# Lounes78/matcha-tts

Hardware: AMD Instinct MI355X
Metric: mel-frames/sec + RTF, text->wav @10 ODE steps, LJSpeech model, 1/2/4/8 GPU (higher is better)
Workload: dtype bf16

## Files before the change

include/matcha_hip.h:

```cpp
#ifndef MATCHA_HIP_H
#define MATCHA_HIP_H

#include <stddef.h>
#include <stdint.h>

#ifdef __cplusplus
extern "C" {
#endif

#define MT_DTYPE_F32 0
#define MT_DTYPE_BF16 1
#define MT_SOLVER_EULER 0
#define MT_SOLVER_MIDPOINT 1

const char* mt_last_error(void);
int mt_abi_version(void);
int mt_build_experiments(void);
int mt_sched_count(void);
int mt_sched_get(int i, int* rec, int* wait, int* wait_first, int cap);

typedef struct mt_encoder mt_encoder;
int mt_encoder_create(int n_vocab, int n_channels, int filter_channels, int n_heads, int n_layers, int kernel_size,
                      int n_spks, int spk_emb_dim, int dp_filter_channels, int dp_kernel_size, int prenet, int dtype,
                      mt_encoder** out);
// ... 132 lines not shown
int mtt_softmax_bwd(const float* p, const float* dp, const float* kmask, const float* qmask, int BH, int H, int Tq,
                    int Tk, float scale, float* ds, void* stream);
int mtt_rope(float* x, int B, int T, int H, int dh, int d, const float* theta, int inverse, void* stream);
int mtt_embed_fwd(const int64_t* ids, size_t ntok, const float* table, int C, float scale, float* out, void* stream);
int mtt_embed_bwd(const int64_t* ids, size_t ntok, const float* dout, int V, int C, float scale, float* dtable,
                  void* stream);
int mtt_adam(float* p, const float* g, float* m, float* v, size_t n, const float* gscale, float lr, float beta1,
             float beta2, float eps, int step, void* stream);
int mtt_clip_factor(const float* sumsq, float max_norm, float inv_world, float* out, float* norm_out, void* stream);
int mtt_unscale(float* g, size_t n, float inv_scale, float* found, float* scratch, void* stream);

size_t mt_op_conv1d_workspace_bytes(int dtype, int cin, int cout, int k, int stride, int transposed);
int mt_op_conv1d(int dtype, const void* x, int B, int Tin, int cin, const float* W, const float* bias,
                 int cout, int k, int stride, int pad, int dil, int transposed, float slope, void* y,
                 int Tout, void* ws, size_t ws_bytes, void* stream);
int mt_op_conv1d_tile(int variant, int dtype, const void* x, int B, int Tin, int cin, const float* W,
                      const float* bias, int cout, int k, int stride, int pad, int dil, int transposed,
                      float slope, void* y, int Tout, void* ws, size_t ws_bytes, void* stream);
size_t mt_op_vconv_workspace_bytes(int cin, int cout, int k);
int mt_op_vconv(const void* x, int B, int L, int cin, const float* W, const float* bias, int cout, int k, int dil,
                int ef, const void* resid, void* y, void* y2, float slope, float div, const int32_t* lens, int pack,
                void* ws, size_t ws_bytes, void* stream);
int mt_vconv_set_rbconv(int enable);
int mt_vconv_set_ct(int enable);
int mt_vpair_set_kernels(int mask);
int mt_vocoder_set_post_fold(int enable);
int mt_vconv_set_actin(int enable);
int mt_ffn_set(int enable);
int mt_ffn_set_min_frames(int frames);
int mt_decoder_set_kernels(int mask);
int mt_op_attention(int dtype, const void* qkv, const float* mask, void* out, int B, int T, int heads,
                    void* stream);

#define MT_PROBE_RBFUSE_C64 1
#define MT_PROBE_RBFUSE_C32 2
#define MT_PROBE_VCONV 3
#define MT_PROBE_VCONV_DEC 4
int mt_probe_start(int site, int max_launches);
int mt_probe_pause(int paused);
int mt_probe_detail(int cap, double* ms, double* flops, double* bytes, int* tags);
int mt_probe_stop(int* launches, double* total_ms, double* flops, double* bytes, double peak_flops, double peak_bw,
                  double* roof_ms);

#define MT_VCONV_LOG_FIELDS 11
int mt_vconv_log_start(int capacity);
int mt_vconv_log_stop(int32_t* records, int capacity);
// ... 7 lines not shown
```

matcha-tts_amd/csrc/mt_capi.hip:

```cpp
#include <string.h>

#include <new>

#include "../../include/matcha_hip.h"
#include "mt_ffn.h"
#include "mt_model.h"
#include "mt_vconv.h"
#include "mt_vpair.h"
#include "mt_probe.h"
#include "mt_train.h"

namespace mt {
const char* last_error();
int denoise(const float* audio, int B, int L, const float* bias_spec, float strength, float* out, void* ws,
            size_t ws_bytes, hipStream_t st, const int* lens = nullptr, int lmul = 1);
size_t denoise_workspace_bytes(int B, int L);
int vconv_exp_flags();
int rbconv_exp_flags();
int ffn_exp_flags();
int vpair_exp_flags();
int stft_magnitude(const float* audio, int B, int L, float* mag, hipStream_t st);
int log_mel(const float* audio, int B, int L, const float* basis, float mean, float stdv, float* mel, hipStream_t st);
}

// ... 351 lines not shown
  mt::ConvArgs a = mt::gemm_args(g, (const char*)ws, B, Tin);
  MT_REQUIRE(a.Tout == Tout, "op_conv1d: Tout %d != expected %d", Tout, a.Tout);
  a.x0 = x;
  a.y = y;
  a.slope = slope;
  return mt::launch_conv_op(dtype, slope >= 0.f ? mt::PF_LRELU : 0, a, st, variant);
}
int mt_op_conv1d(int dtype, const void* x, int B, int Tin, int cin, const float* W, const float* bias,
                 int cout, int k, int stride, int pad, int dil, int transposed, float slope, void* y, int Tout,
                 void* ws, size_t ws_bytes, void* stream) {
  return mt_op_conv1d_tile(-1, dtype, x, B, Tin, cin, W, bias, cout, k, stride, pad, dil, transposed, slope, y,
                           Tout, ws, ws_bytes, stream);
}
size_t mt_op_vconv_workspace_bytes(int cin, int cout, int k) {
  mt::Packer pk;
  mt::GemmW g = mt::make_conv(cout, cin, k, 1, 0, 1, {0}, 1, 2, pk);
  pk.take(mt::vconv_packed_bytes(cin, cout, k));
  pk.take(256);
  pk.take(4096);
  (void)g;
  return pk.off;
}
int mt_vconv_set_rbconv(int enable) { return mt::rbconv_set(enable); }
int mt_vconv_set_ct(int enable) { return mt::vconv_set_ct(enable); }
int mt_ffn_set(int enable) { return mt::ffn_set(enable); }
int mt_vconv_set_actin(int enable) { return mt::rbconv_actin_set(enable); }
int mt_ffn_set_min_frames(int frames) { return mt::ffn_set_min_frames(frames); }
int mt_decoder_set_kernels(int mask) { return mt::dec_set_kernels(mask); }
int mt_op_vconv(const void* x, int B, int L, int cin, const float* W, const float* bias, int cout, int k, int dil,
                int ef, const void* resid, void* y, void* y2, float slope, float div, const int32_t* lens, int pack,
                void* ws, size_t ws_bytes, void* stream) {
  MT_REQUIRE(x && W && bias && y && ws, "op_vconv: null argument");
  MT_REQUIRE(mt::vconv_supported(cin, cout, k, dil, 1), "op_vconv: unsupported conv %dx%d k%d d%d", cin, cout, k, dil);
  hipStream_t st = (hipStream_t)stream;
  mt::Packer pk;
  mt::GemmW g = mt::make_conv(cout, cin, k, 1, dil * (k - 1) / 2, dil, {0}, 1, 2, pk);
  const size_t v_off = pk.take(mt::vconv_packed_bytes(cin, cout, k));
  const size_t z_off = pk.take(256);
  const size_t t_off = pk.take(4096);
  MT_REQUIRE(ws_bytes >= pk.off, "op_vconv: workspace %zu < %zu", ws_bytes, pk.off);
  const float* params[2] = {W, bias};
  char* P = (char*)ws;
  int rc;
  if (pack) {
    if ((rc = mt::pack_gemm(g, MT_DTYPE_BF16, params, P, st))) return rc;
    if ((rc = mt::vconv_repack(P + g.w_off, g.Mpad, g.taps, g.cin_pad, cin, cout, P + v_off, st))) return rc;
// ... 155 lines not shown
```

matcha-tts_amd/csrc/mt_ragged.h:

```cpp
#pragma once
#include "mt_common.h"

namespace mt {

constexpr int RAG_MAXB = 512;
constexpr int RAG_LDS = 2 * RAG_MAXB * 4;

__device__ __forceinline__ void rag_build(int* tc, int* lv, const int* lens, int lmul, int Lpad, int extra, int cap,
                                          int B, int BN, int tid) {
  if (tid >= 64) return;
  const int per = (B + 63) >> 6, b0 = tid * per;
  int s = 0;
  for (int i = 0; i < per; ++i) {
    const int b = b0 + i;
    if (b < B) {
      const int L = min(max(lens[b] * lmul, 0), Lpad);
      const int nc = min(max(L + extra, 0), cap);
      s += (nc + BN - 1) / BN;
    }
  }
  int x = s;
#pragma unroll
  for (int o = 1; o < 64; o <<= 1) {
    const int v = __shfl_up(x, o, 64);
    if (tid >= o) x += v;
  }
  int run = x - s;
  for (int i = 0; i < per; ++i) {
    const int b = b0 + i;
    if (b < B) {
      const int L = min(max(lens[b] * lmul, 0), Lpad);
      const int nc = min(max(L + extra, 0), cap);
      run += (nc + BN - 1) / BN;
      tc[b] = run;
      lv[b] = L;
    }
  }
}

__device__ __forceinline__ int rag_find(const int* tc, int B, int r) {
  int lo = 0, hi = B - 1;
  while (lo < hi) {
    const int mid = (lo + hi) >> 1;
    if (tc[mid] > r) hi = mid;
    else lo = mid + 1;
  }
  return lo;
}

__device__ __forceinline__ int rag_first(const int* tc, int b) { return b > 0 ? tc[b - 1] : 0; }

struct RagTile {
  int b, n0, lv;
};
struct RagWalk {
// ... 13 lines not shown
```

matcha-tts_amd/csrc/mt_rbconv.hip:

```cpp
#include <algorithm>
#include <cstdlib>
#include <type_traits>

#include "mt_probe.h"
#include "mt_ragged.h"
#include "mt_ts.h"
#include "mt_vconv.h"

#ifndef RB_ACTIN_NV
#define RB_ACTIN_NV 0
#endif

#ifndef RB_RAGWALK
#define RB_RAGWALK 1
#endif

#ifndef RB_EPI_AT
#define RB_EPI_AT 2
#endif

#ifndef RB_DMA_AT
#define RB_DMA_AT 1
#endif

#ifndef RB_BUF
#define RB_BUF 7
#endif

#ifndef RB_LMAX
#define RB_LMAX 1
#endif

#ifndef RB_EXP
#define RB_EXP 0
#endif

namespace mt {

namespace {
constexpr int RBM = 128, RBN = 256, RNT = 512;
constexpr int RWSLOT = RBM * 128;
constexpr int RNW = 4;
constexpr int RXROWS = RBN + 64;
constexpr int RXBUF = RXROWS * 128;
constexpr int RX_OFF = RNW * RWSLOT;
constexpr int RBIAS_OFF = RX_OFF + 2 * RXBUF;
constexpr int RRAG_OFF = RBIAS_OFF + 256 * 4;
constexpr int RLDS = RRAG_OFF + RAG_LDS;
static_assert(RLDS <= 160 * 1024, "LDS budget");
constexpr int RFN = 4, RWNC = 64;

template <int LW>
struct RbStage {
// ... 136 lines not shown
      for (int i = 0; i < XPW; ++i) {
        if (i * TX / XPW != part) continue;
        const int j = wave + LW * i;
        buf_lds16(xr, (unsigned)(xlane + (f0 + 8 * j) * C * 2), 0u, dst + j * 1024);
      }
    } else {
#pragma unroll
      for (int i = 0; i < XPW; ++i) {
        if (i * TX / XPW != part) continue;
        const int j = wave + LW * i;
        const int r = 8 * j + lrow;
        const int q = lp ^ (r & 6);
        const int f = f0 + r;
        const bool ok = r < R && f >= 0 && f < Lx;
        const char* src = ok ? xb + (size_t)f * C * 2 + q * 16 : reinterpret_cast<const char*>(a.zero) + q * 16;
        rb_glds16(src, dst + j * 1024);
      }
    }
  };

  f32x4 acc[4][RFN];

  const int g4 = lane >> 4, l16 = lane & 15;
  auto swap16 = [](uint32_t& x, uint32_t& y) {
    const auto r = __builtin_amdgcn_permlane16_swap(x, y, false, false);
    x = r[0];
    y = r[1];
  };
  const int ch16 = wm * 64 + (g4 & 1) * 16 + (g4 >> 1) * 8;
  u32x4 rv[2][RFN], yv[2][RFN];
  auto epi_loads = [&](const Tile& tl) __attribute__((always_inline)) {
    const size_t rowbase = (size_t)tl.b * L;
#pragma unroll
    for (int fp = 0; fp < 2; ++fp)
#pragma unroll
      for (int fn = 0; fn < RFN; ++fn) {
        const int n = min(tl.n0 + wn * RWNC + fn * 16 + l16, L - 1);
        const size_t o = (rowbase + n) * C + tl.m0 + ch16 + fp * 32;
        if constexpr ((RB_EXP & 1) != 0) {
          rv[fp][fn] = yv[fp][fn] = u32x4{(uint32_t)o, 0u, 0u, 0u};
          continue;
        }
        if constexpr ((EF & VE_RESID) != 0) rv[fp][fn] = *reinterpret_cast<const u32x4*>(a.resid + o);
        if constexpr ((EF & VE_ACCUM) != 0) yv[fp][fn] = *reinterpret_cast<const u32x4*>(a.y + o);
      }
  };
  auto epilogue = [&](const Tile& tl, bool real) __attribute__((always_inline)) {
    const unsigned ylim = (unsigned)L * (unsigned)(C * 2) - (unsigned)(tl.m0 * 2);
    const auto yr = buf_rsrc(a.y + (size_t)tl.b * L * C + tl.m0, ylim);
    const auto y2r = buf_rsrc(((EF & VE_DUAL) ? a.y2 : a.y) + (size_t)tl.b * L * C + tl.m0, ylim);
#pragma unroll
    for (int fp = 0; fp < 2; ++fp)
#pragma unroll
      for (int fn = 0; fn < RFN; ++fn) {
        uint32_t rx0 = 0, rx1 = 0, ry0 = 0, ry1 = 0, yx0 = 0, yx1 = 0, yy0 = 0, yy1 = 0;
        if constexpr ((EF & VE_RESID) != 0) {
          rx0 = rv[fp][fn][0], rx1 = rv[fp][fn][1], ry0 = rv[fp][fn][2], ry1 = rv[fp][fn][3];
          swap16(rx0, ry0);
          swap16(rx1, ry1);
        }
        if constexpr ((EF & VE_ACCUM) != 0) {
          yx0 = yv[fp][fn][0], yx1 = yv[fp][fn][1], yy0 = yv[fp][fn][2], yy1 = yv[fp][fn][3];
          swap16(yx0, yy0);
          swap16(yx1, yy1);
        }
        uint32_t o1[2][2], o2[2][2];
#pragma unroll
        for (int h = 0; h < 2; ++h) {
          const int fm = 2 * fp + h;
          const int m = tl.m0 + wm * 64 + fm * 16 + 4 * g4;
          const f32x4 bias4 = *reinterpret_cast<const f32x4*>(smem + RBIAS_OFF + 4 * m);
          const uint32_t rr[2] = {h ? ry0 : rx0, h ? ry1 : rx1};
          const uint32_t yy[2] = {h ? yy0 : yx0, h ? yy1 : yx1};
#pragma unroll
          for (int u = 0; u < 2; ++u) {
            f32x2 v = f32x2{acc[fm][fn][2 * u], acc[fm][fn][2 * u + 1]} + f32x2{bias4[2 * u], bias4[2 * u + 1]};
            if constexpr ((EF & VE_RESID) != 0) v = v + unpk_bf16(rr[u]);
            if constexpr ((EF & VE_ACCUM) != 0) v = unpk_bf16(yy[u]) + v;
            if constexpr ((EF & VE_DIV) != 0) v = f32x2{div_rn(v.x, a.div, 1.f / a.div), div_rn(v.y, a.div, 1.f / a.div)};
            const uint32_t rb = pk_bf16(v);
            uint32_t av = 0u;
            if constexpr (RB_LMAX) av = (EF & VE_ACT) ? lrelu_pk_f(v, a.slope) : (EF & VE_DUAL) ? lrelu_pk(rb, a.slope) : 0u;
            else av = (EF & VE_ACT) ? lrelu_pk_f_sel(v, a.slope) : (EF & VE_DUAL) ? lrelu_pk_sel(rb, a.slope) : 0u;
            o1[h][u] = (EF & VE_ACT) ? av : rb;
            o2[h][u] = av;
          }
        }
        swap16(o1[0][0], o1[1][0]);
        swap16(o1[0][1], o1[1][1]);
        const int n = tl.n0 + wn * RWNC + fn * 16 + l16;
        if constexpr ((RB_BUF & 4) != 0) {
          const unsigned vo = (unsigned)((n * C + ch16 + fp * 32) * 2);
          if constexpr ((EF & VE_Y2ONLY) == 0)
            __builtin_amdgcn_raw_buffer_store_b128(u32x4{o1[0][0], o1[0][1], o1[1][0], o1[1][1]}, yr, vo, 0, 0);
          if constexpr ((EF & VE_DUAL) != 0 && (RB_EXP & 2) == 0) {
            swap16(o2[0][0], o2[1][0]);
            swap16(o2[0][1], o2[1][1]);
            __builtin_amdgcn_raw_buffer_store_b128(u32x4{o2[0][0], o2[0][1], o2[1][0], o2[1][1]}, y2r, vo, 0, 0);
          }
          continue;
        }
        const bool ok = real && n < L;
        const size_t o = ((size_t)tl.b * L + n) * C + tl.m0 + ch16 + fp * 32;
        if constexpr ((EF & VE_Y2ONLY) == 0)
          *reinterpret_cast<u32x4*>(ok ? a.y + o : a.trash + 8 * lane) = u32x4{o1[0][0], o1[0][1], o1[1][0], o1[1][1]};
        if constexpr ((EF & VE_DUAL) != 0 && (RB_EXP & 2) == 0) {
          swap16(o2[0][0], o2[1][0]);
          swap16(o2[0][1], o2[1][1]);
          *reinterpret_cast<u32x4*>(ok ? a.y2 + o : a.trash + 8 * lane) = u32x4{o2[0][0], o2[0][1], o2[1][0], o2[1][1]};
        }
      }
  };

  struct Frag {
    bf16x8 A[4], B[RFN];
  };
  const int ha = l16 & 6;
  const char* pa0 = smem + (wm * 64 + l16) * 128;
  const int rbl = wn * RWNC + l16;
  auto read_frag = [&](Frag& F, int ks, int slot, int xbuf, int tap) __attribute__((always_inline)) {
    int lb = rbl, la = 0;
    asm volatile("" : "+v"(lb), "+v"(la));
    const char* pa = pa0 + la + slot * RWSLOT;
    const int rb0 = lb + tap * dil;
    const int hb = rb0 & 6;
    const char* pb = smem + RX_OFF + xbuf * RXBUF + rb0 * 128;
    const int oa = ((ks * 4 + g4) ^ ha) * 16, ob = ((ks * 4 + g4) ^ hb) * 16;
#pragma unroll
    for (int f = 0; f < 4; ++f) F.A[f] = *reinterpret_cast<const bf16x8*>(pa + f * 2048 + oa);
#pragma unroll
    for (int f = 0; f < RFN; ++f) F.B[f] = *reinterpret_cast<const bf16x8*>(pb + f * 2048 + ob);
  };
  auto act_pass = [&](int buf) __attribute__((always_inline)) {
// ... 223 lines not shown
```

matcha-tts_amd/csrc/mt_vconv.h:

```cpp
#pragma once
#include <type_traits>

#include "mt_common.h"

namespace mt {

enum : int {
  VE_RESID = 1,
  VE_ACCUM = 2,
  VE_DIV = 4,
  VE_ACT = 8,
  VE_DUAL = 16,
  VE_LN = 32,
  VE_SNAKE = 64,
  VE_MASK = 128,
  VE_GNSTATS = 256,
  VE_ROWSTATS = 512,
  VE_LNP = 1024,
  VE_RELU = 2048,
  VE_PMASK = 4096,
  VE_ACTIN = 16384,
  VE_Y2ONLY = 32768,
  VE_POST = 131072,
  VE_SPLIT6 = 65536,
// ... 128 lines not shown
  int xcd_tiles;
};

__device__ __forceinline__ float2 ln_merge4(f32x4 p01, f32x4 p23, float eps) {
#pragma clang fp contract(off)
  const float mean = 0.25f * ((p01[0] + p01[2]) + (p23[0] + p23[2]));
  const float d0 = p01[0] - mean, d1 = p01[2] - mean, d2 = p23[0] - mean, d3 = p23[2] - mean;
  const float m2 = (p01[1] + p01[3]) + (p23[1] + p23[3]) + 64.f * ((d0 * d0 + d1 * d1) + (d2 * d2 + d3 * d3));
  return float2{mean, rsqrtf(m2 * (1.f / 256.f) + eps)};
}

int vconv_gn_parts(int B, int L, int M);
int vconv_gn_parts_max(int L);
int vconv_gnres_min_frames();

bool vconv_supported(int cin, int cout, int k, int dil, int stride);
size_t vconv_packed_bytes(int cin, int cout, int k);
int vconv_repack(const void* src, int Mpad0, int taps, int cin_pad, int cin, int cout, void* dst, hipStream_t st,
                 int cin_src = -1);
int launch_vconv(int ef, const VConvArgs& a, hipStream_t st);
bool rbconv_handles(int ef, const VConvArgs& a);
int launch_rbconv(int ef, const VConvArgs& a, int G, hipStream_t st);
int rbconv_set(int enable);
int rbconv_actin_set(int enable);
int rbconv_actin_on();
int vconv_set_ct(int enable);
int vconv_path_id();
bool vconv_supported_f32(int cin, int cout, int k, int stride);
size_t vconv_packed_bytes_f32(int cin, int cout, int k);
int vconv_repack_f32(const void* src, int Mpad0, int taps, int cin_pad, int cin, int cout, void* dst, hipStream_t st);
size_t vconv_packed_bytes_split6(int cin, int cout, int k);
int vconv_repack_split6(const void* src, int Mpad0, int taps, int cin_pad, int cin, int cout, void* dst, hipStream_t st);
__device__ __forceinline__ void split3_bf16(float v, bf16& h1, bf16& h2, bf16& h3) {
  h1 = (bf16)v;
  const float r1 = v - (float)h1;
  h2 = (bf16)r1;
  h3 = (bf16)(r1 - (float)h2);
}
int vconv_repack_s2(const void* src, int cin_pad, int C, int cout, void* dst, hipStream_t st);
int vconv_wsum(const void* img, int cin, int taps, int cout, float* wsum, hipStream_t st);

}
```

matcha-tts_amd/csrc/mt_vconv.hip:

```cpp
#include <algorithm>
#include <climits>
#include <cstdlib>
#include <type_traits>

#include "mt_misc.h"
#include "mt_probe.h"
#include "mt_ragged.h"
#include "mt_vconv.h"

namespace mt {

namespace {
constexpr int BN = 256, NT = 512;
constexpr int MMAX = 1024;
constexpr int BMP = 64;
template <int BM_, bool K1_, int NPAR_, int BN_ = BN>
struct VT {
  static constexpr int BM = BM_, TBN = BN_;
  static constexpr int WAVES_M = BM / 64, WAVES_N = 8 / WAVES_M;
  static constexpr int WNC = TBN / WAVES_N;
  static constexpr int FN = WNC / 16;
  static_assert(WNC % 16 == 0, "a wave covers whole 16-frame fragments");
  static constexpr int WSLOT = BM * 128;
  static constexpr int NWW = BM / 64;
// ... 1250 lines not shown
  if (tf != BN) ntiles = (long)a.B * ((a.L + tf - 1) / tf) * (a.Mpad / BM);
  const int G = (int)std::min<long>(ntiles, cu_count());
  a.xcd_tiles = a.xcd_tiles && ntiles <= 3L * G;
  MT_REQUIRE(!(ef & VE_GNSTATS) || a0.gn_parts == 0 || a0.gn_parts == ((a.L + tf - 1) / tf) * (8 / (BM / 64)),
             "vconv: caller expects %d GroupNorm partial slots, the launch writes a different count", a0.gn_parts);
  {
    const int bn = k1 ? tf1 : (BM == 64 ? (bm64_128 ? 128 : 384) : tf);
    const int rec[VCLOG_FIELDS] = {ef, BM, bn, (int)k1, (int)ntiles, G, a.taps, a.M, a.cin, a.B, a.L};
    vclog_record(rec);
#if defined(VCONV_TS)
    ts_assign(a, rec);
#endif
  }
  const double flops = 2.0 * a.M * a.cin * a.taps * (double)a.B * a.Lout;
  const double bytes = 2.0 * a.B * ((double)a.L * a.cin + (double)a.Lout * a.M) + 2.0 * a.M * a.cin * a.taps;
  const int site = a.probe ? a.probe : PROBE_VCONV;
  const bool probed = !k1 && site > 0;
  if ((ef & VE_Y2ONLY) && !(!k1 && !placed && BM == 128 && rbconv_handles(ef, a))) ef &= ~VE_Y2ONLY;
  MT_REQUIRE(!(ef & VE_ACTIN) || (!k1 && !placed && BM == 128 && rbconv_handles(ef, a)),
             "vconv: VE_ACTIN launch not taken by mt_rbconv (cin %d M %d k %d d %d B %d): stage_actin and the launch "
             "arguments disagree", a.cin, a.M, a.taps, a.dil, a.B);
  if (!k1 && !placed && BM == 128 && rbconv_handles(ef, a)) {
    if (probed) probe_begin(site, st);
    const int rc = launch_rbconv(ef, a, G, st);
    if (rc) return rc;
    if (probed) probe_end(site, st, flops, bytes, PROBE_TAG_RBCONV);
    return 0;
  }
  if (probed) probe_begin(site, st);
#define MT_VCASE(E)                                                                                \
  case E:                                                                                          \
    if (BM == 128) hipLaunchKernelGGL((vconv_kernel<E, 128, false>), dim3(G), dim3(NT), 0, st, a); \
    else hipLaunchKernelGGL((vconv_kernel<E, 64, false, BN64>), dim3(G), dim3(NT), 0, st, a);     \
    break;
#define MT_VCASE_H(E)                                                                                  \
  case E:                                                                                              \
    if (tf == 128) hipLaunchKernelGGL((vconv_kernel<E, 128, false, 128>), dim3(G), dim3(NT), 0, st, a); \
    else if (tf == 192) hipLaunchKernelGGL((vconv_kernel<E, 128, false, 192>), dim3(G), dim3(NT), 0, st, a); \
    else if (BM == 128) hipLaunchKernelGGL((vconv_kernel<E, 128, false>), dim3(G), dim3(NT), 0, st, a); \
    else hipLaunchKernelGGL((vconv_kernel<E, 64, false, BN64>), dim3(G), dim3(NT), 0, st, a);          \
    break;
#define MT_VCASE1(E)                                                                                    \
  case E:                                                                                               \
    if (tf1 == 128) {                                                                                   \
      if (BM == 128) hipLaunchKernelGGL((vconv_kernel<E, 128, true, 128>), dim3(G), dim3(NT), 0, st, a); \
      else hipLaunchKernelGGL((vconv_kernel<E, 64, true, 128>), dim3(G), dim3(NT), 0, st, a);           \
    } else if (tf1 == 192) {                \
// ... 101 lines not shown
```

matcha-tts_amd/matcha_hip/_lib.py:

```python
from __future__ import annotations

import ctypes
import os
from ctypes import POINTER, c_char_p, c_double, c_float, c_int, c_int64, c_size_t, c_uint, c_void_p

PKG_DIR = os.path.dirname(os.path.dirname(os.path.abspath(__file__)))
LIB_PATH = os.path.join(PKG_DIR, "libmatcha_hip.so")

DTYPE_F32 = 0
DTYPE_BF16 = 1
SOLVER_EULER = 0
SOLVER_MIDPOINT = 1

P = c_void_p

SIGNATURES = {
    "mt_last_error": (c_char_p, []),
    "mt_abi_version": (c_int, []),
    "mt_build_experiments": (c_int, []),
    "mt_sched_count": (c_int, []),
    "mt_sched_get": (c_int, [c_int, P, P, P, c_int]),
    "mt_encoder_create": (c_int, [c_int, c_int, c_int, c_int, c_int, c_int, c_int, c_int, c_int, c_int, c_int, c_int,
                                  POINTER(c_void_p)]),
    "mt_encoder_destroy": (None, [P]),
# ... 43 lines not shown
    "mt_vocoder_ragged_supported": (c_int, [P]),
    "mt_durations": (c_int, [P, P, c_float, c_int, c_int, P, P, P, P]),
    "mt_durations_scaled": (c_int, [P, P, P, c_int, c_int, P, P, P, P]),
    "mt_alignment": (c_int, [P, P, c_int, c_int, c_int, P, c_int, P, P, P, P]),
    "mt_denorm_crop": (c_int, [P, P, P, c_int, c_int, c_int, c_int, P, P]),
    "mt_denoise_workspace_bytes": (c_size_t, [c_int, c_int]),
    "mt_denoise": (c_int, [P, c_int, c_int, P, c_float, P, P, c_size_t, P]),
    "mt_denoise_ragged": (c_int, [P, c_int, c_int, P, c_int, P, c_float, P, P, c_size_t, P]),
    "mt_maximum_path_workspace_bytes": (c_size_t, [c_int, c_int, c_int]),
    "mt_decoder_step_times_workspace_bytes": (c_size_t, [P, c_int, c_int]),
    "mt_decoder_step_times": (c_int, [P, P, P, P, P, P, P, c_int, c_int, P, P, c_size_t, P]),
    "mt_maximum_path": (c_int, [P, P, P, c_int, c_int, c_int, P, P, c_size_t, P]),
    "mt_stft_magnitude": (c_int, [P, c_int, c_int, P, P]),
    "mt_log_mel": (c_int, [P, c_int, c_int, P, c_float, c_float, P, P]),
    "mt_op_conv1d_workspace_bytes": (c_size_t, [c_int, c_int, c_int, c_int, c_int, c_int]),
    "mt_op_conv1d": (c_int, [c_int, P, c_int, c_int, c_int, P, P, c_int, c_int, c_int, c_int, c_int,
                             c_int, c_float, P, c_int, P, c_size_t, P]),
    "mt_op_conv1d_tile": (c_int, [c_int, c_int, P, c_int, c_int, c_int, P, P, c_int, c_int, c_int, c_int, c_int,
                                  c_int, c_float, P, c_int, P, c_size_t, P]),
    "mt_op_vconv_workspace_bytes": (c_size_t, [c_int, c_int, c_int]),
    "mt_op_vconv": (c_int, [P, c_int, c_int, c_int, P, P, c_int, c_int, c_int, c_int, P, P, P, c_float, c_float,
                            P, c_int, P, c_size_t, P]),
    "mt_vconv_set_rbconv": (c_int, [c_int]),
    "mt_vconv_set_ct": (c_int, [c_int]),
    "mt_vpair_set_kernels": (c_int, [c_int]),
    "mt_vocoder_set_post_fold": (c_int, [c_int]),
    "mt_ffn_set": (c_int, [c_int]),
    "mt_vconv_set_actin": (c_int, [c_int]),
    "mt_ffn_set_min_frames": (c_int, [c_int]),
    "mt_decoder_set_kernels": (c_int, [c_int]),
    "mt_op_attention": (c_int, [c_int, P, P, P, c_int, c_int, c_int, P]),
    "mt_probe_start": (c_int, [c_int, c_int]),
    "mt_probe_pause": (c_int, [c_int]),
    "mt_probe_detail": (c_int, [c_int, P, P, P, P]),
    "mt_probe_stop": (c_int, [P, P, P, P, c_double, c_double, P]),
    "mtt_gemm": (c_int, [c_int, c_int, c_int, c_int, c_int, c_float, P, c_int, c_int64, P, c_int, c_int64, c_float,
                         P, c_int, c_int64, c_int, P, P, P, c_size_t, P]),
    "mtt_gemm_ex": (c_int, [c_int, c_int, c_int, c_int, c_int, c_int, c_float, P, c_int, c_int64, P, c_int, c_int64,
                            c_float, P, c_int, c_int64, c_int, P, P, P, c_size_t, P]),
    "mtt_gemm_workspace_bytes": (c_size_t, [c_int, c_int, c_int, c_int]),
    "mtt_im2col": (c_int, [P, P, c_int, c_int, c_int, c_int, c_int, c_int, c_int, c_int, P, P]),
    "mtt_col2im": (c_int, [P, P, c_int, c_int, c_int, c_int, c_int, c_int, c_int, c_int, P, c_int, P]),
    "mtt_ew": (c_int, [c_int, c_size_t, P, P, P, P, c_float, c_float, c_size_t, c_size_t, c_size_t, c_size_t,
                       c_size_t, c_size_t, c_int, P]),
    "mtt_copy_cols": (c_int, [P, c_int, c_int, P, c_int, c_int, c_int, c_int, c_int, P]),
    "mtt_seq_mask": (c_int, [P, c_int, c_int, P, P]),
# ... 75 lines not shown
```

matcha-tts_amd/matcha_hip/runtime.py:

```python
from __future__ import annotations

import math
import numbers
import time
from ctypes import byref, c_char_p, c_int, c_int64, c_void_p, create_string_buffer
from typing import Dict, List, Optional, Tuple

import torch

from ._lib import (DTYPE_BF16, DTYPE_F32, SOLVER_EULER, SOLVER_MIDPOINT, HipPathError, check, lib,
                   ptr, stream_handle)

_DTYPES = {"fp32": DTYPE_F32, "float32": DTYPE_F32, "f32": DTYPE_F32,
           "bf16": DTYPE_BF16, "bfloat16": DTYPE_BF16,
           "fp32x3": DTYPE_F32}


def dtype_code(precision: str) -> int:
    try:
        return _DTYPES[precision]
    except KeyError:
        raise ValueError(f"precision must be one of {sorted(set(_DTYPES))}, got {precision!r}")


# ... 594 lines not shown
    return int(lib().mt_vocoder_set_post_fold(int(bool(enable))))


def set_ffn(mode) -> int:
    return int(lib().mt_ffn_set(int(mode)))


def set_ffn_min_frames(frames: int) -> int:
    return int(lib().mt_ffn_set_min_frames(int(frames)))


def set_decoder_kernels(mask: int) -> int:
    return int(lib().mt_decoder_set_kernels(int(mask)))


def set_rbconv_actin(enable: bool) -> bool:
    return bool(lib().mt_vconv_set_actin(int(bool(enable))))


def set_rbconv(enable: bool) -> bool:
    return bool(lib().mt_vconv_set_rbconv(int(bool(enable))))


def op_attention(qkv: torch.Tensor, mask: torch.Tensor, heads: int, precision="fp32") -> torch.Tensor:
    require_gpu(qkv, mask, what="op_attention")
    dt = dtype_code(precision)
    et = torch.bfloat16 if dt == DTYPE_BF16 else torch.float32
    qkv = qkv.to(et).contiguous()
    B, T, _ = qkv.shape
    out = torch.empty((B, T, heads * 64), dtype=et, device=qkv.device)
    mask = f32c(mask.reshape(B, T))
    check(lib().mt_op_attention(dt, ptr(qkv), ptr(mask), ptr(out), B, T, heads, stream_handle(qkv.device)),
          "op_attention")
    return out


PROBE_RBFUSE_C64, PROBE_RBFUSE_C32, PROBE_VCONV, PROBE_VCONV_DEC = 1, 2, 3, 4


def probe_start(site: int, max_launches: int) -> None:
    check(lib().mt_probe_start(int(site), int(max_launches)), "probe_start")


def probe_pause(paused: bool) -> None:
    check(lib().mt_probe_pause(int(bool(paused))), "probe_pause")

# ... 2 lines not shown


def probe_detail(cap: int = 4096) -> List[Dict[str, float]]:
    from ctypes import c_double
    ms, fl, by, tg = (c_double * cap)(), (c_double * cap)(), (c_double * cap)(), (c_int * cap)()
    n = lib().mt_probe_detail(int(cap), ms, fl, by, tg)
    if n < 0:
        check(n, "probe_detail")
    return [{"ms": ms[i], "flops": fl[i], "bytes": by[i], "kind": PROBE_TAGS[tg[i]]} for i in range(n)]


def probe_stop(peak_flops: float = 2.5e15, peak_bw: float = 8.0e12) -> Dict[str, float]:
    from ctypes import c_double
    n, ms, fl, by, roof = c_int(0), c_double(0), c_double(0), c_double(0), c_double(0)
    check(lib().mt_probe_stop(byref(n), byref(ms), byref(fl), byref(by), float(peak_flops), float(peak_bw),
                              byref(roof)), "probe_stop")
    return {"launches": n.value, "ms": ms.value, "flops": fl.value, "bytes": by.value, "roof_ms": roof.value}


VCONV_LOG_FIELDS = ("ef", "bm", "bn", "k1", "ntiles", "grid", "taps", "M", "cin", "B", "L")
PROJ_LOG = 0x20000
UNI_LOG_PART, UNI_LOG_VEC, UNI_LOG_APPLY = 0x40000, 0x80000, 0xC0000
FFN_LOG = 0x400000
LOG_CONV, LOG_AUX = 1, 2


def vconv_log_select(families: int) -> int:
    return int(lib().mt_vconv_log_select(int(families)))


def vconv_log_start(capacity: int = 65536) -> None:
    check(lib().mt_vconv_log_start(int(capacity)), "vconv_log_start")


def vconv_log_stop(capacity: int = 65536) -> List[Dict[str, int]]:
    buf = (c_int * (capacity * len(VCONV_LOG_FIELDS)))()
    n = lib().mt_vconv_log_stop(buf, int(capacity))
    k = len(VCONV_LOG_FIELDS)
    return [dict(zip(VCONV_LOG_FIELDS, buf[i * k:(i + 1) * k])) for i in range(n)]
```

Before: 815,700.

## Add weight-stationary persistent conv kernel for 128-channel vocoder resblock convs

Adds a new persistent HIP kernel that keeps the full 128x128xK conv weights in registers across tiles and loops over ragged time tiles per CU. It double-buffers input rows in LDS and overlaps the next tile's load with the current compute. By default it is used for k=7 resblock convs with residual, accumulate or dual epilogues. The epilogue is factored into a shared header, and ragged tile counts gain an optional rounding. This is meant to remove repeated weight loads and per-tile launch overhead, at the cost of high register pressure and one block per CU.

Result: no change. 818,300 (median of 6 runs) (+0.3%).

```diff
diff --git a/include/matcha_hip.h b/include/matcha_hip.h
--- a/include/matcha_hip.h
+++ b/include/matcha_hip.h
@@ -178,6 +178,7 @@
                 int ef, const void* resid, void* y, void* y2, float slope, float div, const int32_t* lens, int pack,
                 void* ws, size_t ws_bytes, void* stream);
 int mt_vconv_set_rbconv(int enable);
+int mt_vconv_set_wsconv(int mode);
 int mt_vconv_set_ct(int enable);
 int mt_vpair_set_kernels(int mask);
 int mt_vocoder_set_post_fold(int enable);
diff --git a/matcha-tts_amd/csrc/mt_capi.hip b/matcha-tts_amd/csrc/mt_capi.hip
--- a/matcha-tts_amd/csrc/mt_capi.hip
+++ b/matcha-tts_amd/csrc/mt_capi.hip
@@ -397,6 +397,7 @@
   return pk.off;
 }
 int mt_vconv_set_rbconv(int enable) { return mt::rbconv_set(enable); }
+int mt_vconv_set_wsconv(int mode) { return mt::wsconv_set(mode); }
 int mt_vconv_set_ct(int enable) { return mt::vconv_set_ct(enable); }
 int mt_ffn_set(int enable) { return mt::ffn_set(enable); }
 int mt_vconv_set_actin(int enable) { return mt::rbconv_actin_set(enable); }
diff --git a/matcha-tts_amd/csrc/mt_ragged.h b/matcha-tts_amd/csrc/mt_ragged.h
--- a/matcha-tts_amd/csrc/mt_ragged.h
+++ b/matcha-tts_amd/csrc/mt_ragged.h
@@ -7,7 +7,7 @@
 constexpr int RAG_LDS = 2 * RAG_MAXB * 4;
 
 __device__ __forceinline__ void rag_build(int* tc, int* lv, const int* lens, int lmul, int Lpad, int extra, int cap,
-                                          int B, int BN, int tid) {
+                                          int B, int BN, int tid, int round = 1) {
   if (tid >= 64) return;
   const int per = (B + 63) >> 6, b0 = tid * per;
   int s = 0;
@@ -15,7 +15,7 @@
     const int b = b0 + i;
     if (b < B) {
       const int L = min(max(lens[b] * lmul, 0), Lpad);
-      const int nc = min(max(L + extra, 0), cap);
+      const int nc = min((max(L + extra, 0) + round - 1) / round * round, cap);
       s += (nc + BN - 1) / BN;
     }
   }
@@ -30,7 +30,7 @@
     const int b = b0 + i;
     if (b < B) {
       const int L = min(max(lens[b] * lmul, 0), Lpad);
-      const int nc = min(max(L + extra, 0), cap);
+      const int nc = min((max(L + extra, 0) + round - 1) / round * round, cap);
       run += (nc + BN - 1) / BN;
       tc[b] = run;
       lv[b] = L;
diff --git a/matcha-tts_amd/csrc/mt_rbconv.hip b/matcha-tts_amd/csrc/mt_rbconv.hip
--- a/matcha-tts_amd/csrc/mt_rbconv.hip
+++ b/matcha-tts_amd/csrc/mt_rbconv.hip
@@ -4,6 +4,7 @@
 
 #include "mt_probe.h"
 #include "mt_ragged.h"
+#include "mt_rbepi.h"
 #include "mt_ts.h"
 #include "mt_vconv.h"
 
@@ -25,10 +26,6 @@
 
 #ifndef RB_BUF
 #define RB_BUF 7
-#endif
-
-#ifndef RB_LMAX
-#define RB_LMAX 1
 #endif
 
 #ifndef RB_EXP
@@ -211,11 +208,6 @@
   f32x4 acc[4][RFN];
 
   const int g4 = lane >> 4, l16 = lane & 15;
-  auto swap16 = [](uint32_t& x, uint32_t& y) {
-    const auto r = __builtin_amdgcn_permlane16_swap(x, y, false, false);
-    x = r[0];
-    y = r[1];
-  };
   const int ch16 = wm * 64 + (g4 & 1) * 16 + (g4 >> 1) * 8;
   u32x4 rv[2][RFN], yv[2][RFN];
   auto epi_loads = [&](const Tile& tl) __attribute__((always_inline)) {
@@ -242,62 +234,24 @@
     for (int fp = 0; fp < 2; ++fp)
 #pragma unroll
       for (int fn = 0; fn < RFN; ++fn) {
-        uint32_t rx0 = 0, rx1 = 0, ry0 = 0, ry1 = 0, yx0 = 0, yx1 = 0, yy0 = 0, yy1 = 0;
-        if constexpr ((EF & VE_RESID) != 0) {
-          rx0 = rv[fp][fn][0], rx1 = rv[fp][fn][1], ry0 = rv[fp][fn][2], ry1 = rv[fp][fn][3];
-          swap16(rx0, ry0);
-          swap16(rx1, ry1);
-        }
-        if constexpr ((EF & VE_ACCUM) != 0) {
-          yx0 = yv[fp][fn][0], yx1 = yv[fp][fn][1], yy0 = yv[fp][fn][2], yy1 = yv[fp][fn][3];
-          swap16(yx0, yy0);
-          swap16(yx1, yy1);
-        }
-        uint32_t o1[2][2], o2[2][2];
-#pragma unroll
-        for (int h = 0; h < 2; ++h) {
-          const int fm = 2 * fp + h;
-          const int m = tl.m0 + wm * 64 + fm * 16 + 4 * g4;
-          const f32x4 bias4 = *reinterpret_cast<const f32x4*>(smem + RBIAS_OFF + 4 * m);
-          const uint32_t rr[2] = {h ? ry0 : rx0, h ? ry1 : rx1};
-          const uint32_t yy[2] = {h ? yy0 : yx0, h ? yy1 : yx1};
-#pragma unroll
-          for (int u = 0; u < 2; ++u) {
-            f32x2 v = f32x2{acc[fm][fn][2 * u], acc[fm][fn][2 * u + 1]} + f32x2{bias4[2 * u], bias4[2 * u + 1]};
-            if constexpr ((EF & VE_RESID) != 0) v = v + unpk_bf16(rr[u]);
-            if constexpr ((EF & VE_ACCUM) != 0) v = unpk_bf16(yy[u]) + v;
-            if constexpr ((EF & VE_DIV) != 0) v = f32x2{div_rn(v.x, a.div, 1.f / a.div), div_rn(v.y, a.div, 1.f / a.div)};
-            const uint32_t rb = pk_bf16(v);
-            uint32_t av = 0u;
-            if constexpr (RB_LMAX) av = (EF & VE_ACT) ? lrelu_pk_f(v, a.slope) : (EF & VE_DUAL) ? lrelu_pk(rb, a.slope) : 0u;
-            else av = (EF & VE_ACT) ? lrelu_pk_f_sel(v, a.slope) : (EF & VE_DUAL) ? lrelu_pk_sel(rb, a.slope) : 0u;
-            o1[h][u] = (EF & VE_ACT) ? av : rb;
-            o2[h][u] = av;
-          }
-        }
-        swap16(o1[0][0], o1[1][0]);
-        swap16(o1[0][1], o1[1][1]);
+        u32x4 out1, out2;
+        rb_epi_pair<EF>(a, acc[2 * fp][fn], acc[2 * fp + 1][fn], rv[fp][fn], yv[fp][fn],
+                        smem + RBIAS_OFF + 4 * (tl.m0 + wm * 64 + fp * 32 + 4 * g4), out1, out2);
         const int n = tl.n0 + wn * RWNC + fn * 16 + l16;
         if constexpr ((RB_BUF & 4) != 0) {
           const unsigned vo = (unsigned)((n * C + ch16 + fp * 32) * 2);
           if constexpr ((EF & VE_Y2ONLY) == 0)
-            __builtin_amdgcn_raw_buffer_store_b128(u32x4{o1[0][0], o1[0][1], o1[1][0], o1[1][1]}, yr, vo, 0, 0);
-          if constexpr ((EF & VE_DUAL) != 0 && (RB_EXP & 2) == 0) {
-            swap16(o2[0][0], o2[1][0]);
-            swap16(o2[0][1], o2[1][1]);
-            __builtin_amdgcn_raw_buffer_store_b128(u32x4{o2[0][0], o2[0][1], o2[1][0], o2[1][1]}, y2r, vo, 0, 0);
-          }
+            __builtin_amdgcn_raw_buffer_store_b128(out1, yr, vo, 0, 0);
+          if constexpr ((EF & VE_DUAL) != 0 && (RB_EXP & 2) == 0)
+            __builtin_amdgcn_raw_buffer_store_b128(out2, y2r, vo, 0, 0);
           continue;
         }
         const bool ok = real && n < L;
         const size_t o = ((size_t)tl.b * L + n) * C + tl.m0 + ch16 + fp * 32;
         if constexpr ((EF & VE_Y2ONLY) == 0)
-          *reinterpret_cast<u32x4*>(ok ? a.y + o : a.trash + 8 * lane) = u32x4{o1[0][0], o1[0][1], o1[1][0], o1[1][1]};
-        if constexpr ((EF & VE_DUAL) != 0 && (RB_EXP & 2) == 0) {
-          swap16(o2[0][0], o2[1][0]);
-          swap16(o2[0][1], o2[1][1]);
-          *reinterpret_cast<u32x4*>(ok ? a.y2 + o : a.trash + 8 * lane) = u32x4{o2[0][0], o2[0][1], o2[1][0], o2[1][1]};
-        }
+          *reinterpret_cast<u32x4*>(ok ? a.y + o : a.trash + 8 * lane) = out1;
+        if constexpr ((EF & VE_DUAL) != 0 && (RB_EXP & 2) == 0)
+          *reinterpret_cast<u32x4*>(ok ? a.y2 + o : a.trash + 8 * lane) = out2;
       }
   };
 
diff --git a/matcha-tts_amd/csrc/mt_rbepi.h b/matcha-tts_amd/csrc/mt_rbepi.h
--- /dev/null
+++ b/matcha-tts_amd/csrc/mt_rbepi.h
@@ -0,0 +1,61 @@
+#pragma once
+#include "mt_vconv.h"
+
+#ifndef RB_LMAX
+#define RB_LMAX 1
+#endif
+
+namespace mt {
+
+__device__ __forceinline__ void rb_swap16(uint32_t& x, uint32_t& y) {
+  const auto r = __builtin_amdgcn_permlane16_swap(x, y, false, false);
+  x = r[0];
+  y = r[1];
+}
+
+template <int EF>
+__device__ __forceinline__ void rb_epi_pair(const VConvArgs& a, const f32x4& acc0, const f32x4& acc1, const u32x4& rv,
+                                            const u32x4& yv, const char* bias, u32x4& out1, u32x4& out2) {
+  uint32_t rx0 = 0, rx1 = 0, ry0 = 0, ry1 = 0, yx0 = 0, yx1 = 0, yy0 = 0, yy1 = 0;
+  if constexpr ((EF & VE_RESID) != 0) {
+    rx0 = rv[0], rx1 = rv[1], ry0 = rv[2], ry1 = rv[3];
+    rb_swap16(rx0, ry0);
+    rb_swap16(rx1, ry1);
+  }
+  if constexpr ((EF & VE_ACCUM) != 0) {
+    yx0 = yv[0], yx1 = yv[1], yy0 = yv[2], yy1 = yv[3];
+    rb_swap16(yx0, yy0);
+    rb_swap16(yx1, yy1);
+  }
+  uint32_t o1[2][2], o2[2][2];
+#pragma unroll
+  for (int h = 0; h < 2; ++h) {
+    const f32x4& acc = h ? acc1 : acc0;
+    const f32x4 bias4 = *reinterpret_cast<const f32x4*>(bias + 64 * h);
+    const uint32_t rr[2] = {h ? ry0 : rx0, h ? ry1 : rx1};
+    const uint32_t yy[2] = {h ? yy0 : yx0, h ? yy1 : yx1};
+#pragma unroll
+    for (int u = 0; u < 2; ++u) {
+      f32x2 v = f32x2{acc[2 * u], acc[2 * u + 1]} + f32x2{bias4[2 * u], bias4[2 * u + 1]};
+      if constexpr ((EF & VE_RESID) != 0) v = v + unpk_bf16(rr[u]);
+      if constexpr ((EF & VE_ACCUM) != 0) v = unpk_bf16(yy[u]) + v;
+      if constexpr ((EF & VE_DIV) != 0) v = f32x2{div_rn(v.x, a.div, 1.f / a.div), div_rn(v.y, a.div, 1.f / a.div)};
+      const uint32_t rb = pk_bf16(v);
+      uint32_t av = 0u;
+      if constexpr (RB_LMAX) av = (EF & VE_ACT) ? lrelu_pk_f(v, a.slope) : (EF & VE_DUAL) ? lrelu_pk(rb, a.slope) : 0u;
+      else av = (EF & VE_ACT) ? lrelu_pk_f_sel(v, a.slope) : (EF & VE_DUAL) ? lrelu_pk_sel(rb, a.slope) : 0u;
+      o1[h][u] = (EF & VE_ACT) ? av : rb;
+      o2[h][u] = av;
+    }
+  }
+  rb_swap16(o1[0][0], o1[1][0]);
+  rb_swap16(o1[0][1], o1[1][1]);
+  out1 = u32x4{o1[0][0], o1[0][1], o1[1][0], o1[1][1]};
+  if constexpr ((EF & VE_DUAL) != 0) {
+    rb_swap16(o2[0][0], o2[1][0]);
+    rb_swap16(o2[0][1], o2[1][1]);
+    out2 = u32x4{o2[0][0], o2[0][1], o2[1][0], o2[1][1]};
+  }
+}
+
+}
diff --git a/matcha-tts_amd/csrc/mt_vconv.h b/matcha-tts_amd/csrc/mt_vconv.h
--- a/matcha-tts_amd/csrc/mt_vconv.h
+++ b/matcha-tts_amd/csrc/mt_vconv.h
@@ -174,6 +174,10 @@
 bool rbconv_handles(int ef, const VConvArgs& a);
 int launch_rbconv(int ef, const VConvArgs& a, int G, hipStream_t st);
 int rbconv_set(int enable);
+bool wsconv_handles(int ef, const VConvArgs& a);
+int launch_wsconv(int ef, const VConvArgs& a, int cus, hipStream_t st);
+int wsconv_set(int mode);
+constexpr int WS_LOG = 0x800000;
 int rbconv_actin_set(int enable);
 int rbconv_actin_on();
 int vconv_set_ct(int enable);
diff --git a/matcha-tts_amd/csrc/mt_vconv.hip b/matcha-tts_amd/csrc/mt_vconv.hip
--- a/matcha-tts_amd/csrc/mt_vconv.hip
+++ b/matcha-tts_amd/csrc/mt_vconv.hip
@@ -1296,7 +1296,7 @@
              "arguments disagree", a.cin, a.M, a.taps, a.dil, a.B);
   if (!k1 && !placed && BM == 128 && rbconv_handles(ef, a)) {
     if (probed) probe_begin(site, st);
-    const int rc = launch_rbconv(ef, a, G, st);
+    const int rc = wsconv_handles(ef, a) ? launch_wsconv(ef, a, cu_count(), st) : launch_rbconv(ef, a, G, st);
     if (rc) return rc;
     if (probed) probe_end(site, st, flops, bytes, PROBE_TAG_RBCONV);
     return 0;
diff --git a/matcha-tts_amd/csrc/mt_wsconv.hip b/matcha-tts_amd/csrc/mt_wsconv.hip
--- /dev/null
+++ b/matcha-tts_amd/csrc/mt_wsconv.hip
@@ -0,0 +1,312 @@
+#include <algorithm>
+#include <cstdlib>
+
+#include "mt_probe.h"
+#include "mt_ragged.h"
+#include "mt_rbepi.h"
+#include "mt_vconv.h"
+
+#ifndef WS_PF
+#define WS_PF 2
+#endif
+#ifndef WS_LDAT
+#define WS_LDAT 6
+#endif
+#ifndef WS_ACTB
+#define WS_ACTB 6
+#endif
+
+namespace mt {
+
+namespace {
+constexpr int WC = 128, WN = 192, WNT = 256, WFN = 4, WNB = WN / (16 * WFN);
+constexpr int WRND = 256;
+constexpr int WROWS = WN + 64;
+constexpr int WP = 288;
+constexpr int WXBUF = WROWS * WP;
+constexpr int WPC = WXBUF / 1024 / 4;
+static_assert(WXBUF == 4 * WPC * 1024 && WPC % 9 == 0, "whole pieces per wave, whole 32-row groups");
+constexpr int WBIAS_OFF = 2 * WXBUF;
+constexpr int WRAG_OFF = WBIAS_OFF + WC * 4;
+constexpr int WLDS = WRAG_OFF + RAG_LDS;
+static_assert(WLDS <= 160 * 1024, "LDS budget");
+static_assert((16 * (WFN - 1) + 64) * WP + 128 + 64 + 16 <= 65536, "ds_read immediate offset");
+
+template <int EF>
+constexpr int ws_nst() {
+  return WFN * ((EF & VE_DUAL) && !(EF & VE_Y2ONLY) ? 2 : 1);
+}
+
+template <class T>
+__device__ __forceinline__ void ws_pin(T& x) {
+  asm volatile("" : "+v"(x));
+}
+
+__device__ __forceinline__ void ws_barrier() {
+  __builtin_amdgcn_sched_barrier(0);
+  asm volatile("" ::: "memory");
+  __builtin_amdgcn_s_barrier();
+  asm volatile("" ::: "memory");
+  __builtin_amdgcn_sched_barrier(0);
+}
+}
+
+template <int EF, int K>
+__global__ __launch_bounds__(WNT) void wsconv_kernel(VConvArgs a) {
+  constexpr int NS = WC / 32 * K;
+  constexpr bool ACTIN = (EF & VE_ACTIN) != 0;
+  constexpr int NST = ws_nst<EF>();
+  __shared__ __attribute__((aligned(1024))) char smem[WLDS];
+  const int tid = threadIdx.x, lane = tid & 63;
+  const int wave = __builtin_amdgcn_readfirstlane(tid >> 6);
+  const int g4 = lane >> 4, l16 = lane & 15;
+  const int dil = a.dil, L = a.L;
+  const int ntn = (L + WN - 1) / WN;
+  const bool rag = a.lens != nullptr;
+  int* rtc = reinterpret_cast<int*>(smem + WRAG_OFF);
+  int* rlv = rtc + RAG_MAXB;
+  if (rag) rag_build(rtc, rlv, a.lens, a.lmul, L, 0, L, a.B, WN, tid, WRND);
+  for (int i = tid; i < WC; i += WNT) reinterpret_cast<float*>(smem + WBIAS_OFF)[i] = a.bias[i];
+  __syncthreads();
+  const int ntiles = __builtin_amdgcn_readfirstlane(rag ? rtc[a.B - 1] : a.B * ntn);
+  const int G = gridDim.x, g = blockIdx.x;
+  const int xcd = g & 7, lw = g >> 3;
+  const int gx = (G - xcd + 7) >> 3;
+  const int sx = xcd * (G >> 3) + min(xcd, G & 7);
+  const int xt0 = (int)((long)ntiles * sx / G), xt1 = (int)((long)ntiles * (sx + gx) / G);
+  const bool xmaj = a.xcd_tiles != 0;
+  const int gl = xmaj ? xt0 + lw : (G % 8 == 0) ? (g % 8) * (G / 8) + g / 8 : g;
+  const int gstep = xmaj ? gx : G;
+  const int nmine = xmaj ? (gl < xt1 ? (xt1 - gl + gx - 1) / gx : 0) : (gl < ntiles ? (ntiles - gl + G - 1) / G : 0);
+  if (nmine == 0) return;
+
+  struct Tile {
+    int b, n0, lx;
+  };
+  RagWalk walk;
+  auto tile_of = [&](int ti) __attribute__((always_inline)) {
+    Tile tl;
+    const int r = __builtin_amdgcn_readfirstlane(gl + min(ti, nmine - 1) * gstep);
+    if (rag) {
+      const RagTile rt = walk.at(rtc, rlv, a.B, WN, r);
+      tl.b = rt.b, tl.n0 = rt.n0, tl.lx = rt.lv;
+    } else {
+      tl.b = r / ntn;
+      tl.n0 = (r - tl.b * ntn) * WN;
+      tl.lx = L;
+    }
+    tl.b = __builtin_amdgcn_readfirstlane(tl.b);
+    tl.n0 = __builtin_amdgcn_readfirstlane(tl.n0);
+    tl.lx = __builtin_amdgcn_readfirstlane(tl.lx);
+    return tl;
+  };
+
+  bf16x8 A[2][NS];
+  {
+    const char* wl = reinterpret_cast<const char*>(a.w) + (wave * 32 + l16) * 128 + g4 * 16;
+    vc_for<0, NS>([&](auto sc) {
+      constexpr int s = decltype(sc)::value;
+      constexpr int ct = s / 2, ks = s & 1;
+#pragma unroll
+      for (int h = 0; h < 2; ++h) A[h][s] = *reinterpret_cast<const bf16x8*>(wl + (ct * 128 + h * 16) * 128 + ks * 64);
+    });
+    vc_for<0, NS>([&](auto sc) {
+      constexpr int s = decltype(sc)::value;
+      ws_pin(A[0][s]);
+      ws_pin(A[1][s]);
+    });
+  }
+
+  auto issue_rows = [&](const Tile& tl, int buf) __attribute__((always_inline)) {
+    const char* xb = reinterpret_cast<const char*>(a.x) + (size_t)tl.b * L * (WC * 2);
+    const auto xr = buf_rsrc(xb, (unsigned)tl.lx * (unsigned)(WC * 2));
+    int xo = buf * WXBUF + wave * (WPC * 1024);
+    asm volatile("" : "+s"(xo));
+    int ln = lane;
+    asm volatile("" : "+v"(ln));
+    const int row0 = tl.n0 - a.pad + wave * (WPC / 9 * 32);
+#pragma unroll
+    for (int i = 0; i < WPC; ++i) {
+      const int u = (i % 9) * 64 + ln;
+      const int q = (u * 3641) >> 16, r = u - q * 18;
+      const unsigned vo = (unsigned)((row0 + (i / 9) * 32 + q) * (WC * 2) + r * 16);
+      buf_lds16(xr, r < 16 ? vo : 0x80000000u, 0u, smem + xo + i * 1024);
+    }
+  };
+  auto act_pass = [&](int buf) __attribute__((always_inline)) {
+    int bo = buf * WXBUF + wave * (WPC * 1024) + lane * 16;
+    asm volatile("" : "+v"(bo));
+    static_assert(WPC % WS_ACTB == 0, "whole batches");
+#pragma unroll
+    for (int i0 = 0; i0 < WPC; i0 += WS_ACTB) {
+      u32x4 v[WS_ACTB];
+#pragma unroll
+      for (int i = 0; i < WS_ACTB; ++i) v[i] = *reinterpret_cast<const u32x4*>(smem + bo + (i0 + i) * 1024);
+#pragma unroll
+      for (int i = 0; i < WS_ACTB; ++i) {
+#pragma unroll
+        for (int w = 0; w < 4; ++w) v[i][w] = lrelu_pk(v[i][w], a.slope);
+        *reinterpret_cast<u32x4*>(smem + bo + (i0 + i) * 1024) = v[i];
+      }
+      __builtin_amdgcn_sched_barrier(0);
+    }
+  };
+
+  const int ch16 = wave * 32 + (g4 & 1) * 16 + (g4 >> 1) * 8;
+  const int dstep = dil * WP;
+  auto block = [&](const Tile& tl, int buf, int nb) __attribute__((always_inline)) {
+    f32x4 acc[2][WFN];
+    bf16x8 Bf[WS_PF + 1][WFN];
+    u32x4 rv[WFN], yv[WFN];
+    const auto rr = buf_rsrc(((EF & VE_RESID) ? a.resid : a.y) + (size_t)tl.b * L * WC, (unsigned)L * (unsigned)(WC * 2));
+    const unsigned ylim = (unsigned)min((tl.lx + WRND - 1) / WRND * WRND, L) * (unsigned)(WC * 2);
+    const auto yr = buf_rsrc(a.y + (size_t)tl.b * L * WC, ylim);
+    const auto y2r = buf_rsrc(((EF & VE_DUAL) ? a.y2 : a.y) + (size_t)tl.b * L * WC, ylim);
+    const int nl = tl.n0 + nb * 64 + l16;
+    int bo = buf * WXBUF + (nb * 64 + l16) * WP + g4 * 16;
+    asm volatile("" : "+v"(bo));
+    int bt[2];
+    auto read_slice = [&](auto sc) __attribute__((always_inline)) {
+      constexpr int s = decltype(sc)::value;
+      constexpr int st = s / 2, c = st / K, t = st % K, ks = s & 1;
+      if constexpr (ks == 0) {
+        bt[st & 1] = bo + t * dstep;
+        ws_pin(bt[st & 1]);
+      }
+      const char* pb = smem + bt[st & 1] + c * 128 + ks * 64;
+#pragma unroll
+      for (int fn = 0; fn < WFN; ++fn) Bf[s % (WS_PF + 1)][fn] = *reinterpret_cast<const bf16x8*>(pb + fn * 16 * WP);
+    };
+    vc_for<0, WS_PF>(read_slice);
+    __builtin_amdgcn_sched_group_barrier(0x100, WS_PF * WFN, 0);
+    vc_for<0, NS>([&](auto sc) {
+      constexpr int s = decltype(sc)::value;
+      if constexpr (s + WS_PF < NS) read_slice(std::integral_constant<int, s + WS_PF>{});
+      if constexpr (s == (K == 7 ? 0 : NS - 1 - WS_LDAT) && (EF & (VE_RESID | VE_ACCUM)) != 0) {
+#pragma unroll
+        for (int fn = 0; fn < WFN; ++fn) {
+          const unsigned vo = (unsigned)(((nl + fn * 16) * WC + ch16) * 2);
+          if constexpr ((EF & VE_RESID) != 0) rv[fn] = __builtin_amdgcn_raw_buffer_load_b128(rr, vo, 0, 0);
+          if constexpr ((EF & VE_ACCUM) != 0) yv[fn] = __builtin_amdgcn_raw_buffer_load_b128(yr, vo, 0, 0);
+        }
+      }
+#pragma unroll
+      for (int h = 0; h < 2; ++h)
+#pragma unroll
+        for (int fn = 0; fn < WFN; ++fn)
+          acc[h][fn] = mfma16(A[h][s], Bf[s % (WS_PF + 1)][fn], s == 0 ? f32x4{0.f, 0.f, 0.f, 0.f} : acc[h][fn]);
+#pragma unroll
+      for (int i = 0; i < WFN; ++i) {
+        __builtin_amdgcn_sched_group_barrier(0x008, 1, 0);
+        __builtin_amdgcn_sched_group_barrier(0x100, 1, 0);
+      }
+      __builtin_amdgcn_sched_group_barrier(0x008, 2 * WFN - WFN, 0);
+    });
+    __builtin_amdgcn_sched_barrier(0);
+#pragma unroll
+    for (int fn = 0; fn < WFN; ++fn) {
+      u32x4 out1, out2;
+      rb_epi_pair<EF>(a, acc[0][fn], acc[1][fn], rv[fn], yv[fn], smem + WBIAS_OFF + 4 * (wave * 32 + 4 * g4), out1,
+                      out2);
+      const unsigned vo = (unsigned)(((nl + fn * 16) * WC + ch16) * 2);
+      if constexpr ((EF & VE_Y2ONLY) == 0) __builtin_amdgcn_raw_buffer_store_b128(out1, yr, vo, 0, 0);
+      if constexpr ((EF & VE_DUAL) != 0) __builtin_amdgcn_raw_buffer_store_b128(out2, y2r, vo, 0, 0);
+    }
+    __builtin_amdgcn_sched_barrier(0);
+  };
+
+  Tile cur = tile_of(0), nxt = tile_of(1);
+  issue_rows(cur, 0);
+  asm volatile("s_waitcnt vmcnt(0)" ::: "memory");
+  if constexpr (ACTIN) {
+    act_pass(0);
+    asm volatile("s_waitcnt lgkmcnt(0)" ::: "memory");
+  }
+  ws_barrier();
+
+  for (int ti = 0; ti < nmine; ++ti) {
+    const int buf = ti & 1;
+    const bool more = ti + 1 < nmine;
+    for (int nb = 0; nb < WNB; ++nb) {
+      if constexpr (ACTIN) {
+        if (nb == WNB - 1 && more) {
+          vc_wait_vmcnt<NST>();
+          act_pass(buf ^ 1);
+        }
+      }
+      block(cur, buf, nb);
+      if (nb == 0 && more) issue_rows(nxt, buf ^ 1);
+    }
+    vc_wait_vmcnt<NST>();
+    asm volatile("s_waitcnt lgkmcnt(0)" ::: "memory");
+    ws_barrier();
+    cur = nxt;
+    nxt = tile_of(ti + 2);
+  }
+}
+
+namespace {
+int g_ws = -2;
+int ws_knob() {
+  if (g_ws == -2) {
+    const char* e = getenv("MT_WSCONV");
+    g_ws = !e ? -1 : e[0] == '0' ? 0 : 1;
+  }
+  return g_ws;
+}
+bool ws_default(int ef, int taps) {
+  return taps == 7 && (ef == VE_RESID || ef == (VE_RESID | VE_ACCUM) || ef == (VE_RESID | VE_DUAL));
+}
+}
+
+int wsconv_set(int mode) {
+  const int prev = ws_knob();
+  g_ws = mode < 0 ? -1 : mode ? 1 : 0;
+  return prev;
+}
+
+bool wsconv_handles(int ef, const VConvArgs& a) {
+  const int mode = ws_knob();
+  if (mode == 0) return false;
+  const bool eps = ef == VE_ACT || ef == (VE_ACT | VE_ACTIN) || ef == (VE_RESID | VE_DUAL) || ef == VE_RESID ||
+                   ef == (VE_RESID | VE_ACCUM) || ef == (VE_RESID | VE_ACCUM | VE_DIV) ||
+                   ef == (VE_RESID | VE_ACCUM | VE_DIV | VE_DUAL) ||
+                   ef == (VE_RESID | VE_ACCUM | VE_DIV | VE_DUAL | VE_Y2ONLY);
+  if (!(eps && !a.f32 && a.cin == WC && a.M == WC && a.Mpad == WC && a.c0 == WC && (a.taps == 7 || a.taps == 11) &&
+        a.dil >= 1 && (a.taps - 1) * a.dil <= 64 && a.Lout == a.L && a.ldy == a.M && a.yshift == 0 &&
+        a.ylim == a.L * a.M && a.B <= RAG_MAXB))
+    return false;
+  return mode == 1 || ws_default(ef, a.taps);
+}
+
+int launch_wsconv(int ef, const VConvArgs& a0, int cus, hipStream_t st) {
+  VConvArgs a = a0;
+  const long ntiles = (long)a.B * ((a.L + WN - 1) / WN);
+  const int G = (int)std::min<long>(ntiles, cus);
+  a.xcd_tiles = a.xcd_tiles && ntiles <= 3L * G;
+  {
+    const int rec[VCLOG_FIELDS] = {WS_LOG | ef, WC, WN, 0, (int)ntiles, G, a.taps, WC, WC, a.B, a.L};
+    vclog_record(rec, VCLOG_AUX);
+  }
+#define MT_WS_EF(E)                                                                             \
+  case E:                                                                                       \
+    if (a.taps == 7) hipLaunchKernelGGL((wsconv_kernel<E, 7>), dim3(G), dim3(WNT), 0, st, a);   \
+    else hipLaunchKernelGGL((wsconv_kernel<E, 11>), dim3(G), dim3(WNT), 0, st, a);              \
+    break;
+  switch (ef) {
+    MT_WS_EF(VE_ACT)
+    MT_WS_EF(VE_ACT | VE_ACTIN)
+    MT_WS_EF(VE_RESID | VE_DUAL)
+    MT_WS_EF(VE_RESID)
+    MT_WS_EF(VE_RESID | VE_ACCUM)
+    MT_WS_EF(VE_RESID | VE_ACCUM | VE_DIV)
+    MT_WS_EF(VE_RESID | VE_ACCUM | VE_DIV | VE_DUAL)
+    MT_WS_EF(VE_RESID | VE_ACCUM | VE_DIV | VE_DUAL | VE_Y2ONLY)
+    default: set_error("wsconv: epilogue %d", ef); return -1;
+  }
+#undef MT_WS_EF
+  MT_CHECK_HIP(hipGetLastError());
+  return 0;
+}
+
+}
diff --git a/matcha-tts_amd/matcha_hip/_lib.py b/matcha-tts_amd/matcha_hip/_lib.py
--- a/matcha-tts_amd/matcha_hip/_lib.py
+++ b/matcha-tts_amd/matcha_hip/_lib.py
@@ -89,6 +89,7 @@
     "mt_op_vconv": (c_int, [P, c_int, c_int, c_int, P, P, c_int, c_int, c_int, c_int, P, P, P, c_float, c_float,
                             P, c_int, P, c_size_t, P]),
     "mt_vconv_set_rbconv": (c_int, [c_int]),
+    "mt_vconv_set_wsconv": (c_int, [c_int]),
     "mt_vconv_set_ct": (c_int, [c_int]),
     "mt_vpair_set_kernels": (c_int, [c_int]),
     "mt_vocoder_set_post_fold": (c_int, [c_int]),
diff --git a/matcha-tts_amd/matcha_hip/runtime.py b/matcha-tts_amd/matcha_hip/runtime.py
--- a/matcha-tts_amd/matcha_hip/runtime.py
+++ b/matcha-tts_amd/matcha_hip/runtime.py
@@ -640,6 +640,10 @@
     return bool(lib().mt_vconv_set_rbconv(int(bool(enable))))
 
 
+def set_wsconv(mode) -> int:
+    return int(lib().mt_vconv_set_wsconv(-1 if mode is None else int(mode)))
+
+
 def op_attention(qkv: torch.Tensor, mask: torch.Tensor, heads: int, precision="fp32") -> torch.Tensor:
     require_gpu(qkv, mask, what="op_attention")
     dt = dtype_code(precision)
@@ -688,6 +692,7 @@
 PROJ_LOG = 0x20000
 UNI_LOG_PART, UNI_LOG_VEC, UNI_LOG_APPLY = 0x40000, 0x80000, 0xC0000
 FFN_LOG = 0x400000
+WS_LOG = 0x800000
 LOG_CONV, LOG_AUX = 1, 2
 
 
```
